# helgeanl/GP-MPC

Measured on NVIDIA H100. Metric: GP predictions/sec (N train x horizon test, fp64), higher is better.
Workload: dtype f64

## Files before the change

### gp-mpc_b200/csrc/gpmpc.cu

```cuda
#include "../../include/gpmpc.h"

#include <dlfcn.h>
#include <math.h>
#include <stdarg.h>
#include <stdlib.h>
#include <string.h>

#include <algorithm>
#include <type_traits>
#include <vector>

#include <nvtx3/nvToolsExt.h>

#include "common.cuh"
#include "gemm_dmma.cuh"
#include "predict_streamk.cuh"
#include "kernels.cuh"

#define GPMPC_VERSION 100
#define HB 64
#define NX_MAX 32
#define PSK_MAX_CTAS 2048
#define MAX_DEPTH 12
#define LOOKAHEAD_MIN_ROWS 1024
// ... 33 lines not shown
    return true;
}

template <typename T>
struct DevBuf {
    T* p = nullptr;
    size_t cap = 0;
    DevBuf() = default;
    DevBuf(const DevBuf&) = delete;
    DevBuf& operator=(const DevBuf&) = delete;
    ~DevBuf() { cudaFree(p); }
    operator T*() const { return p; }
    int ensure(gpmpc_handle_t h, long long count, const char* name);
};

struct gpmpc_handle_s {
    int N = 0, Nx = 0, Ny = 0, a0 = 0, nloc = 0, Npad = 0, device = 0;
    int nloc_max = 0;
    cudaStream_t st = nullptr;
    cudaEvent_t ev0 = nullptr, ev1 = nullptr;
    cudaStream_t sideSt[MAX_DEPTH] = {nullptr}; cudaEvent_t evA[MAX_DEPTH] = {nullptr}, evB[MAX_DEPTH] = {nullptr}, evT[MAX_DEPTH] = {nullptr}, evS[MAX_DEPTH] = {nullptr};
    long long w2off[MAX_DEPTH + 1] = {0};
    DevBuf<double> dXT, dMu, dY, dHyp, dJit, dHypTmp;
    DevBuf<double> dL, dLi, dW1, dW2;
    DevBuf<double> dAlpha, dTmp, dRes;
    DevBuf<int> dInfo;
    DevBuf<double> dKST, dPart, dPMJ, dSQ, dV, dR, dR2;
    DevBuf<unsigned int> dCnt;
    int psk_ctas = 0, opt_predict_ctas = 0;
    DevBuf<double> dCovV, dCovOut;
    DevBuf<double> dGrD;
    DevBuf<int> dGrI;
    DevBuf<double> dRm;
    DevBuf<double> dUall, dBeta, dPDV, dPH, dGradOut; bool u_valid = false;
    DevBuf<double> dDR, dVD, dPG, dPB2, dPM3, dHessOut;
    DevBuf<double> dG;
    double *dZ = nullptr, *dSigma = nullptr, *dMean = nullptr, *dVar = nullptr, *dJ = nullptr, *dCov = nullptr;
    DevBuf<double> dRoll;
    DevBuf<double> dSmV;
    DevBuf<double> dSmp;
    DevBuf<double> dIn, dOut;
    int Hcap = 0;
    double* hPinned = nullptr; double* dPinnedAlias = nullptr; size_t hPinnedBytes = 0;
    DevBuf<double> dU, dKinv, dGradPart, dGrad;
    DevBuf<double> dLoo;
    bool has_data = false, has_hyper = false, factorized = false;
    DevBuf<double> dEmTr, dEMP, dEmE, dEmF, dEmW, dEmIJ;
    DevBuf<double> dEmMeanPart, dEmPart, dEmLQ, dEmVec, dEmE2, dEmF2;
    DevBuf<double> dEmKinv, dEmGPart, dEmGRec, dEmBB; bool em_kinv_valid = false;
    std::vector<double> hyper;
    std::vector<double> logdet, yalpha;
    std::vector<int> jitter_used;
    int sms = 132;
    int opt_refine = 0, opt_small_tiles = 528;
    nccl_comm_t comm = nullptr; int rank = 0, world = 1;
    DevBuf<double> dPeerBlock; long long peerGsz = 0; int peerHcap = 0; bool peer_ready = false;
    double* peerBase[GPMPC_MAXW] = {nullptr}; bool peerOpened[GPMPC_MAXW] = {false};
    int* dPeerStatus = nullptr; int* hPeerStatus = nullptr;
    unsigned long long peer_step = 0; int opt_peer = 1; double opt_peer_timeout_s = 60.0; int clock_khz = 1980000;
    char err[512] = "";
};

static void set_error(gpmpc_handle_t h, const char* fmt, ...)
{
    va_list ap; va_start(ap, fmt);
    vsnprintf(h ? h->err : g_create_err, 512, fmt, ap);
    va_end(ap);
}

template <typename T>
int DevBuf<T>::ensure(gpmpc_handle_t h, long long count, const char* name)
{
    if ((size_t)count <= cap) return GPMPC_OK;
    if (p) {
        CUDA_TRY(cudaStreamSynchronize(h->st));
        cudaFree(p);
        p = nullptr; cap = 0;
    }
    const size_t bytes = (size_t)count * sizeof(T);
    cudaError_t e = cudaMalloc((void**)&p, bytes);
    if (e != cudaSuccess) {
        p = nullptr;
        set_error(h, "cudaMalloc(%s, %zu bytes) failed: %s", name, bytes, cudaGetErrorString(e));
        return GPMPC_ERR_CUDA;
    }
    e = cudaMemsetAsync(p, 0, bytes, h->st);
    if (e != cudaSuccess) { cudaFree(p); p = nullptr; }
    CUDA_TRY(e);
    cap = (size_t)count;
    return GPMPC_OK;
}

#define ENSURE(buf, count)                                          \
    do {                                                            \
        const int _rc = (buf).ensure(h, (long long)(count), #buf);  \
        if (_rc) return _rc;                                        \
    } while (0)

struct NvtxRange {
    explicit NvtxRange(const char* name) { nvtxRangePushA(name); }
    ~NvtxRange() { nvtxRangePop(); }
};

static inline long long slab(gpmpc_handle_t h) { return (long long)h->Npad * h->Npad; }
static inline long long w2slab(gpmpc_handle_t h) { return h->w2off[MAX_DEPTH]; }

// ... 140 lines not shown
    trmv_lower_kernel<<<g1, 256, 0, h->st>>>(Li, n, slab(h), h->dY + (long long)a * n, n,
                                              h->dTmp + (long long)a * n, n, n);
    CUDA_TRY(cudaGetLastError());
    const int nch = (n + TRT_ROWS - 1) / TRT_ROWS;
    double* P = h->dW1 + (long long)a * w2slab(h);
    dim3 g2(n / 32, nch, batch);
    trmv_lower_T_part_kernel<<<g2, 256, 0, h->st>>>(Li, n, slab(h), h->dTmp + (long long)a * n, n, P, w2slab(h), n);
    CUDA_TRY(cudaGetLastError());
    alpha_logdet_kernel<<<batch, 1024, 0, h->st>>>(P, w2slab(h), nch, h->dL + (long long)a * slab(h), n, slab(h),
                                                   h->dY + (long long)a * n, n, h->dAlpha + (long long)a * n, n, n, h->dRes + 2 * a);
    CUDA_TRY(cudaGetLastError());
    return GPMPC_OK;
}

static int factor_one(gpmpc_handle_t h, int a, const double* dHyp, double jitter, int* used)
{
    double* L = h->dL + (long long)a * slab(h);
    double* Li = h->dLi + (long long)a * slab(h);
    *used = 0;
    for (int attempt = 0; attempt < 2; ++attempt) {
        const double jit = attempt ? jitter : 0.0;
        CUDA_TRY(cudaMemcpyAsync(h->dJit + a, &jit, sizeof(double), cudaMemcpyHostToDevice, h->st));
        CUDA_TRY(cudaMemsetAsync(h->dInfo + a, 0, sizeof(int), h->st));
        {
            int rck = launch_kbuild(h, dHyp, h->dJit + a, L, 1, 0);
            if (rck) return rck;
        }
        int rc = potrf_inv_rec(h, L, Li, slab(h), slab(h), h->dInfo + a, 0, h->Npad, 1);
        if (rc) return rc;
        int info = 0;
        CUDA_TRY(cudaMemcpyAsync(&info, h->dInfo + a, sizeof(int), cudaMemcpyDeviceToHost, h->st));
        CUDA_TRY(cudaStreamSynchronize(h->st));
        if (info == 0) { *used = attempt; return GPMPC_OK; }
        *used = 1 + info;
    }
    return GPMPC_ERR_NOTPD;
}

extern "C" int gpmpc_version(void) { return GPMPC_VERSION; }

extern "C" const char* gpmpc_last_error(gpmpc_handle_t h) { return h ? h->err : g_create_err; }

extern "C" int gpmpc_destroy(gpmpc_handle_t h);

static int create_fill(gpmpc_handle_t h, int N, int N_cap, int Nx, int Ny, int out_begin, int out_count, int device)
{
    h->N = N; h->Nx = Nx; h->Ny = Ny; h->a0 = out_begin; h->nloc = out_count; h->device = device;
    h->nloc_max = out_count; h->world = 1; h->rank = 0;
    h->Npad = (std::max(N, N_cap) + GPMPC_TILE - 1) / GPMPC_TILE * GPMPC_TILE;
    CUDA_TRY(cudaSetDevice(device));
    CUDA_TRY(cudaDeviceGetAttribute(&h->sms, cudaDevAttrMultiProcessorCount, device));
    h->opt_small_tiles = 4 * h->sms;
    h->psk_ctas = PSK_CTAS_PER_SM * h->sms;
    cudaDeviceGetAttribute(&h->clock_khz, cudaDevAttrClockRate, device);
    {
        int lo = 0, hi = 0;
        cudaDeviceGetStreamPriorityRange(&lo, &hi);
        CUDA_TRY(cudaStreamCreateWithPriority(&h->st, cudaStreamNonBlocking, hi));
    }
    CUDA_TRY(cudaEventCreate(&h->ev0));
    CUDA_TRY(cudaEventCreate(&h->ev1));
    const long long np = h->Npad;
    ENSURE(h->dXT, (long long)Nx * np);
    ENSURE(h->dMu, NX_MAX);
    ENSURE(h->dY, (long long)out_count * np);
    ENSURE(h->dHyp, (long long)out_count * (Nx + 2));
    ENSURE(h->dHypTmp, Nx + 2);
    ENSURE(h->dJit, out_count);
    ENSURE(h->dL, out_count * slab(h));
    ENSURE(h->dLi, out_count * slab(h));
    {
        const int nb = h->Npad / 128;
        long long off = 0;
        for (int d = 0; d < MAX_DEPTH; ++d) {
            h->w2off[d] = off;
            const long long nd = (long long)((nb + (1 << d) - 1) >> d) * 128;
            off += nd * nd / 4 + 128;
        }
        h->w2off[MAX_DEPTH] = off;
        int lo = 0, hi = 0;
        cudaDeviceGetStreamPriorityRange(&lo, &hi);
        for (int d = 0; d < MAX_DEPTH; ++d) {
            CUDA_TRY(cudaStreamCreateWithPriority(&h->sideSt[d], cudaStreamNonBlocking, lo));
            CUDA_TRY(cudaEventCreateWithFlags(&h->evA[d], cudaEventDisableTiming));
            CUDA_TRY(cudaEventCreateWithFlags(&h->evB[d], cudaEventDisableTiming));
            CUDA_TRY(cudaEventCreateWithFlags(&h->evT[d], cudaEventDisableTiming));
            CUDA_TRY(cudaEventCreateWithFlags(&h->evS[d], cudaEventDisableTiming));
        }
    }
    ENSURE(h->dW1, out_count * w2slab(h));
    ENSURE(h->dW2, out_count * w2slab(h));
    ENSURE(h->dAlpha, (long long)out_count * np);
    ENSURE(h->dTmp, (long long)out_count * np);
    ENSURE(h->dRes, 2 * out_count);
    ENSURE(h->dInfo, out_count);
    ENSURE(h->dGrad, Nx + 2);
    h->hyper.assign((size_t)out_count * (Nx + 2), 0.0);
    h->logdet.assign(out_count, 0.0); h->yalpha.assign(out_count, 0.0); h->jitter_used.assign(out_count, 0);
    CUDA_TRY(cudaStreamSynchronize(h->st));
    return GPMPC_OK;
}


extern "C" int gpmpc_create(int N, int Nx, int Ny, int out_begin, int out_count, int device, gpmpc_handle_t* out)
{
    return gpmpc_create_reserve(N, N, Nx, Ny, out_begin, out_count, device, out);
// ... 391 lines not shown
        return GPMPC_OK;
    }
    if (!h->factorized) { set_error(h, "gpmpc_get: call gpmpc_factorize first"); return GPMPC_ERR_STATE; }
    switch (what) {
    case GPMPC_GET_CHOL: return extract_to_host(h, h->dL + (long long)al * slab(h), dst, 1);
    case GPMPC_GET_LINV: return extract_to_host(h, h->dLi + (long long)al * slab(h), dst, 1);
    case GPMPC_GET_ALPHA:
        CUDA_TRY(cudaMemcpyAsync(dst, h->dAlpha + (long long)al * h->Npad, h->N * 8, cudaMemcpyDeviceToHost, h->st));
        CUDA_TRY(cudaStreamSynchronize(h->st));
        return GPMPC_OK;
    case GPMPC_GET_LOGDET: dst[0] = h->logdet[al]; return GPMPC_OK;
    case GPMPC_GET_INVK: {
        int rc = compute_kinv(h, al);
        if (rc) return rc;
        return extract_to_host(h, h->dKinv, dst, 2);
    }
    default: set_error(h, "gpmpc_get: unknown selector %d", what); return GPMPC_ERR_ARG;
    }
}

extern "C" int gpmpc_set_option(gpmpc_handle_t h, const char* name, double value)
{
    if (!h || !name) return GPMPC_ERR_ARG;
    if (!strcmp(name, "refine")) { h->opt_refine = value != 0.0; return GPMPC_OK; }
    if (!strcmp(name, "predict_ctas")) {
        const int v = (int)value;
        if (v < 0 || v > PSK_MAX_CTAS) { set_error(h, "predict_ctas must be in [0, %d]", PSK_MAX_CTAS); return GPMPC_ERR_ARG; }
        h->opt_predict_ctas = v; return GPMPC_OK;
    }
    if (!strcmp(name, "peer_timeout_s")) { h->opt_peer_timeout_s = value > 0.0 ? value : 60.0; return GPMPC_OK; }
    if (!strcmp(name, "small_tiles")) { h->opt_small_tiles = (int)value; return GPMPC_OK; }
    if (!strcmp(name, "peer")) { h->opt_peer = value != 0.0; return GPMPC_OK; }
    set_error(h, "unknown option %s", name);
    return GPMPC_ERR_ARG;
}

static inline int ks_chunk(gpmpc_handle_t h)
{
    if (h->Npad < 8192) return 128;
    return (h->nloc >= 2 && h->Nx <= 12) ? 1024 : 512;
}

static inline int ks_blocks(gpmpc_handle_t h) { return (h->Npad + ks_chunk(h) - 1) / ks_chunk(h); }

static inline int round8(int n) { return (n + 7) / 8 * 8; }

static int ensure_rows(gpmpc_handle_t h)
{
    ENSURE(h->dV, (long long)h->nloc * HB * h->Npad);
    ENSURE(h->dR, (long long)h->nloc * HB * h->Npad);
    return GPMPC_OK;
}

static int ensure_predict_bufs(gpmpc_handle_t h, int H)
{
    const long long np = h->Npad, nt = np / 128;
    ENSURE(h->dKST, (long long)h->nloc * HB * np);
    ENSURE(h->dPMJ, (long long)h->nloc * HB * ks_blocks(h) * (h->Nx + 1));
    ENSURE(h->dSQ, (long long)h->nloc * HB * nt);
    ENSURE(h->dCnt, (long long)h->nloc * nt + h->nloc + 1);
    ENSURE(h->dPart, (long long)std::max(h->psk_ctas, h->opt_predict_ctas) * 2 * HB * PSK_BN);
    if (h->opt_refine) {
        int rc = ensure_rows(h);
        if (rc) return rc;
        ENSURE(h->dR2, (long long)h->nloc * HB * np);
    }
    if (H > h->Hcap) {
        h->Hcap = 0;
        h->dZ = h->dSigma = h->dMean = h->dVar = h->dJ = h->dCov = nullptr;
        const long long cap = std::max(H, HB);
        const int nyp = h->nloc_max * h->world;
        const long long Nx = h->Nx, Ny = h->Ny;
        ENSURE(h->dG, (long long)nyp * cap * (Nx + 2));
        ENSURE(h->dIn, cap * Nx + cap * Nx * Nx);
        ENSURE(h->dOut, cap * (2 * Ny + Ny * Nx + Ny * Ny));
        h->dZ = h->dIn; h->dSigma = h->dIn + cap * Nx;
        h->dMean = h->dOut; h->dVar = h->dOut + cap * Ny; h->dJ = h->dOut + 2 * cap * Ny;
        h->dCov = h->dOut + 2 * cap * Ny + cap * Ny * Nx;
        h->Hcap = (int)cap;
    }
    return GPMPC_OK;
}

template <int BM>
static cudaError_t psk_launch_bm(const PredictParams& p, const double* A, long long sA, const double* B, long long sB,
                                 int np, int grid, cudaStream_t st)
{
    constexpr int BYTES = psk_pipe_doubles(BM) * 8 + 2 * PSK_STAGES * 8 + 1024;
    const cudaError_t e = smem_opt_in<predict_streamk_kernel<BM>>(BYTES);
    if (e != cudaSuccess) return e;
    CUtensorMap tmA, tmB;
    if (!tmap_make(&tmA, A, np, BM, np, sA, p.nloc, BM)) return cudaErrorInvalidValue;
    if (!tmap_make(&tmB, B, np, np, np, sB, p.nloc, PSK_BN)) return cudaErrorInvalidValue;
    cudaLaunchConfig_t cfg;
    memset(&cfg, 0, sizeof(cfg));
    cfg.gridDim = dim3(grid); cfg.blockDim = dim3(PSK_THREADS); cfg.dynamicSmemBytes = BYTES; cfg.stream = st;
    cudaLaunchAttribute attr[1];
    attr[0].id = cudaLaunchAttributeProgrammaticStreamSerialization;
    attr[0].val.programmaticStreamSerializationAllowed = 1;
    cfg.attrs = attr; cfg.numAttrs = 1;
    return cudaLaunchKernelEx(&cfg, predict_streamk_kernel<BM>, p, tmA, tmB);
}

static int psk_grid(gpmpc_handle_t h, long long G)
{
    int ctas = h->opt_predict_ctas > 0 ? h->opt_predict_ctas : h->psk_ctas;
    ctas = std::min(ctas, PSK_MAX_CTAS);
    const long long by_work = std::max(1LL, G / 4);
    return (int)std::min<long long>(ctas, h->opt_predict_ctas > 0 ? G : by_work);
}

static cudaError_t psk_launch(gpmpc_handle_t h, const PredictParams& p, const double* A, const double* B)
{
    const long long sA = (long long)HB * h->Npad, sB = slab(h);
    const int np = h->Npad, grid = psk_grid(h, p.G);
    switch (round8(p.Hc)) {
    case 8: return psk_launch_bm<8>(p, A, sA, B, sB, np, grid, h->st);
    case 16: return psk_launch_bm<16>(p, A, sA, B, sB, np, grid, h->st);
    case 24: return psk_launch_bm<24>(p, A, sA, B, sB, np, grid, h->st);
    case 32: return psk_launch_bm<32>(p, A, sA, B, sB, np, grid, h->st);
    case 40: return psk_launch_bm<40>(p, A, sA, B, sB, np, grid, h->st);
    case 48: return psk_launch_bm<48>(p, A, sA, B, sB, np, grid, h->st);
    case 56: return psk_launch_bm<56>(p, A, sA, B, sB, np, grid, h->st);
    default: return psk_launch_bm<64>(p, A, sA, B, sB, np, grid, h->st);
    }
}

static void psk_base(gpmpc_handle_t h, PredictParams& p, int Hc, int upper = 0)
{
    memset(&p, 0, sizeof(p));
    const long long nt = h->Npad / 128;
    p.nloc = h->nloc; p.nt = (int)nt; p.Hc = Hc; p.upper = upper;
    p.ntb = (int)((h->Npad + PSK_BN - 1) / PSK_BN); p.nk = h->Npad / GEMM_BK;
    p.T = psk_steps_per_output(p.ntb, p.nk, upper); p.G = p.T * h->nloc;
    p.part = h->dPart;
    p.tile_cnt = h->dCnt; p.out_cnt = h->dCnt + (long long)h->nloc * nt; p.done_cnt = p.out_cnt + h->nloc;
    p.SQ = h->dSQ;
    p.hyp = h->dHyp; p.hyp_ld = h->Nx + 2; p.Nx = h->Nx;
}

static void psk_finalize(gpmpc_handle_t h, PredictParams& p, int H, int h0)
{
    p.finalize = 1; p.PMJ = h->dPMJ; p.nblk_mj = ks_blocks(h);
    p.Gloc = h->dG; p.slot0 = h->a0; p.Htot = H; p.h0 = h0;
}

static AssembleArgs assemble_args(gpmpc_handle_t h, int H, int method, const double* Sigma, int spp,
                                  double* mean, double* var, double* J, double* cov)
{
    AssembleArgs as;
    memset(&as, 0, sizeof(as));
    as.G = h->dG; as.Ny = h->Ny; as.Nx = h->Nx; as.H = H; as.method_ta = (method == GPMPC_METHOD_TA);
    as.Sigma = Sigma; as.sigma_per_point = spp;
    as.mean = mean; as.var = var; as.J = J; as.cov = cov;
    as.world = 1;
    as.stage_g = (assemble_rows_doubles(H, h->Ny, h->Nx) <= psk_pipe_doubles(round8(std::min(H, HB)))) ? 1 : 0;
    return as;
}

template <int NXP, int CH>
static cudaError_t launch_ks(gpmpc_handle_t h, const double* dZc, int Hc)
{
    const int smem = (NXP + 1) * CH * 8, nblk = ks_blocks(h);
    const cudaError_t e = smem_opt_in<ks_tile_kernel<NXP, CH>>(smem);
    if (e != cudaSuccess) return e;
    dim3 g(nblk, round8(Hc) / 8, h->nloc);
    ks_tile_kernel<NXP, CH><<<g, 256, smem, h->st>>>(h->dXT, h->Npad, h->N, h->Nx, h->dHyp, h->Nx + 2, h->dAlpha, h->Npad,
                                                     dZc, Hc, h->dKST, h->Npad, (long long)HB * h->Npad, h->dPMJ, nblk);
    return cudaGetLastError();
}

template <int CH>
static cudaError_t launch_ks_nx(gpmpc_handle_t h, const double* dZc, int Hc)
{
    const int Nx = h->Nx;
    if (Nx <= 4) return launch_ks<4, CH>(h, dZc, Hc);
    if (Nx <= 6) return launch_ks<6, CH>(h, dZc, Hc);
    if (Nx <= 8) return launch_ks<8, CH>(h, dZc, Hc);
    if (Nx <= 10) return launch_ks<10, CH>(h, dZc, Hc);
    if (Nx <= 12) return launch_ks<12, CH>(h, dZc, Hc);
    if (CH <= 512) {
        if (Nx <= 16) return launch_ks<16, (CH <= 512 ? CH : 512)>(h, dZc, Hc);
        if (Nx <= 24) return launch_ks<24, (CH <= 512 ? CH : 512)>(h, dZc, Hc);
        return launch_ks<32, (CH <= 512 ? CH : 512)>(h, dZc, Hc);
    }
    return cudaErrorInvalidValue;
}
// ... 1206 lines not shown
    CUDA_TRY(cudaIpcGetMemHandle(&mh, h->dPeerBlock));
    static_assert(sizeof(cudaIpcMemHandle_t) == 64, "IPC handle size");
    memcpy(handle64, &mh, 64);
    return GPMPC_OK;
}

extern "C" int gpmpc_peer_attach(gpmpc_handle_t h, const void* handles)
{
    if (!h || !handles) return GPMPC_ERR_ARG;
    if (!h->dPeerBlock) { set_error(h, "gpmpc_peer_attach: call gpmpc_peer_export first"); return GPMPC_ERR_STATE; }
    CUDA_TRY(cudaSetDevice(h->device));
    for (int r = 0; r < h->world; ++r) {
        if (r == h->rank) { h->peerBase[r] = h->dPeerBlock; continue; }
        cudaIpcMemHandle_t mh;
        memcpy(&mh, (const char*)handles + 64 * r, 64);
        void* ptr = nullptr;
        CUDA_TRY(cudaIpcOpenMemHandle(&ptr, mh, cudaIpcMemLazyEnablePeerAccess));
        h->peerBase[r] = (double*)ptr; h->peerOpened[r] = true;
    }
    h->peer_ready = true; h->peer_step = 0;
    return GPMPC_OK;
}

extern "C" int gpmpc_get_size(gpmpc_handle_t h, int* N, int* Nx, int* Ny)
{
    if (!h) return GPMPC_ERR_ARG;
    if (N) *N = h->N;
    if (Nx) *Nx = h->Nx;
    if (Ny) *Ny = h->Ny;
    return GPMPC_OK;
}

extern "C" void* gpmpc_stream(gpmpc_handle_t h) { return h ? (void*)h->st : nullptr; }

extern "C" int gpmpc_synchronize(gpmpc_handle_t h)
{
    if (!h) return GPMPC_ERR_ARG;
    CUDA_TRY(cudaSetDevice(h->device));
    CUDA_TRY(cudaStreamSynchronize(h->st));
    return peer_status_check(h);
}

template <typename Setup>
static int profile_product(gpmpc_handle_t h, const char* fn, int H, const double* out, bool all_outputs, int n_tail,
                           Setup&& setup, std::vector<unsigned long long>& t, int* grid)
{
    if (!h || !out || H < 1 || H > HB) return GPMPC_ERR_ARG;
    int rc = predict_guard(h, fn, GPMPC_METHOD_TA, H);
    if (rc) return rc;
    rc = predict_prepare(h, fn, HB, all_outputs);
    if (rc) return rc;
    PredictParams p;
    psk_base(h, p, H);
    *grid = psk_grid(h, p.G);
    DevBuf<unsigned long long> dbg;
    ENSURE(dbg, (long long)*grid * 2 + n_tail);
    p.dbg = dbg;
    setup(p, dbg + 2 * *grid);
    for (int rep = 0; rep < 2; ++rep) {
        const cudaError_t e = psk_launch(h, p, h->dKST, h->dLi);
        if (e != cudaSuccess) { set_error(h, "%s: %s", fn, cudaGetErrorString(e)); return GPMPC_ERR_CUDA; }
    }
    t.resize((size_t)*grid * 2 + n_tail);
    cudaMemcpyAsync(t.data(), dbg, t.size() * 8, cudaMemcpyDeviceToHost, h->st);
    cudaStreamSynchronize(h->st);
    return GPMPC_OK;
}

extern "C" int gpmpc_profile_balance(gpmpc_handle_t h, int H, double* out4)
{
    std::vector<unsigned long long> t; int grid = 0;
    const int rc = profile_product(h, __func__, H, out4, false, 0, [](PredictParams&, unsigned long long*) {}, t, &grid);
    if (rc) return rc;
    unsigned long long lo = ~0ull, hi = 0; double mn = 1e300, mx = 0.0, sum = 0.0;
    for (int c = 0; c < grid; ++c) {
        const double d = (double)(t[2 * c + 1] - t[2 * c]) * 1e-3;
        mn = std::min(mn, d); mx = std::max(mx, d); sum += d;
        lo = std::min(lo, t[2 * c]); hi = std::max(hi, t[2 * c + 1]);
    }
    out4[0] = mn; out4[1] = mx; out4[2] = sum / grid; out4[3] = (double)(hi - lo) * 1e-3;
    return GPMPC_OK;
}

extern "C" int gpmpc_profile_tail(gpmpc_handle_t h, int H, double* out8)
{
    std::vector<unsigned long long> t; int grid = 0;
    auto setup = [&](PredictParams& p, unsigned long long* tail) {
        psk_finalize(h, p, H, 0);
        p.as = assemble_args(h, H, GPMPC_METHOD_TA, h->dSigma, 0, h->dMean, h->dVar, h->dJ, h->dCov);
        p.as.dbg = tail;
        p.do_assemble = 1;
    };
    const int rc = profile_product(h, __func__, H, out8, true, 8, setup, t, &grid);
    if (rc) return rc;
    unsigned long long lo = ~0ull, hi = 0, hi2 = 0; int cmax = 0;
    for (int c = 0; c < grid; ++c) {
        lo = std::min(lo, t[2 * c]);
        if (t[2 * c + 1] > hi) { hi2 = hi; hi = t[2 * c + 1]; cmax = c; } else hi2 = std::max(hi2, t[2 * c + 1]);
    }
    for (int k = 0; k < 6; ++k) out8[k] = ((double)t[2 * grid + k] - (double)hi2) * 1e-3;
    out8[6] = (double)(hi - lo) * 1e-3;
    out8[7] = (double)(t[2 * cmax + 1] - t[2 * cmax]) * 1e-3;
    return GPMPC_OK;
}

extern "C" int gpmpc_profile_leaf(gpmpc_handle_t h, double* out15)
{
// ... 86 lines not shown
```

### gp-mpc_b200/csrc/predict_streamk.cuh

```cuda
#pragma once
#include "common.cuh"
#include "gemm_dmma.cuh"

#define GPMPC_MAXW 16
#define PSK_CW 8
#define PSK_BN (32 * PSK_CW)
#define PSK_STAGES 5
#define PSK_CTAS_PER_SM 1
#define PSK_THREADS (32 * PSK_CW)

__host__ __device__ constexpr long long psk_pipe_doubles(int bm) { return (long long)PSK_STAGES * (bm + PSK_BN) * GEMM_BK; }


struct PeerArgs {
    double* base[GPMPC_MAXW];
    int world, rank;
    long long goff;
    int flag_idx;
    unsigned long long step;
    long long timeout_clocks;
};

struct AssembleArgs {
    const double* G;
    int Ny, Nx, H, method_ta;
    const double* Sigma; int sigma_per_point;
    double *mean, *var, *J, *cov;
    const unsigned long long* flags;
    int world; unsigned long long step; int* status;
    long long timeout_clocks;
    unsigned long long* dbg;
    int stage_g;
};

struct PredictParams {
    int nloc, nt, Hc;
    int ntb, nk;
    int upper;
    long long T, G;
    double* part;
    unsigned int* tile_cnt;
    unsigned int* out_cnt;
    unsigned int* done_cnt;
    double* SQ;
    double* Vout; long long sV; int ldv;
    int finalize;
    const double* PMJ; int nblk_mj;
    const double* hyp; int hyp_ld, Nx;
    double* Gloc; int slot0, Htot, h0;
    PeerArgs pa; int use_peers, publish;
    AssembleArgs as; int do_assemble;
    unsigned long long* dbg;
};

__device__ __forceinline__ void tail_stamp(unsigned long long* dbg, int k, int tid)
{
    if (dbg && tid == 0) { unsigned long long t; asm volatile("mov.u64 %0, %%globaltimer;" : "=l"(t)); dbg[k] = t; }
}

template <bool WARP>
__device__ __forceinline__ void assemble_point(const AssembleArgs& A, int h, double* sh, int tid, int nth)
{
    const int Ny = A.Ny, Nx = A.Nx, H = A.H;
    double* Jh = sh; double* JS = sh + Ny * Nx; double* vh = sh + 2 * Ny * Nx;
    for (int idx = tid; idx < Ny * Nx; idx += nth) {
        const int a = idx / Nx, d = idx % Nx;
        const double v = __ldcg(A.G + (((long long)a) * H + h) * (Nx + 2) + 2 + d);
        Jh[idx] = v;
        if (A.J) A.J[((long long)h * Ny + a) * Nx + d] = v;
    }
    for (int a = tid; a < Ny; a += nth) {
        const double* g = A.G + (((long long)a) * H + h) * (Nx + 2);
        const double m = __ldcg(g), v = __ldcg(g + 1);
        if (A.mean) A.mean[(long long)h * Ny + a] = m;
        if (A.var) A.var[(long long)h * Ny + a] = v;
        vh[a] = v;
    }
    if (WARP) __syncwarp(); else __syncthreads();
    if (A.cov) {
        if (A.method_ta) {
            const double* Sg = A.Sigma + (A.sigma_per_point ? (long long)h * Nx * Nx : 0);
            for (int idx = tid; idx < Ny * Nx; idx += nth) {
                const int a = idx / Nx, e = idx % Nx;
                double s = 0.0;
                for (int d = 0; d < Nx; ++d) s = fma(Jh[a * Nx + d], Sg[d * Nx + e], s);
                JS[idx] = s;
            }
            if (WARP) __syncwarp(); else __syncthreads();
        }
        for (int idx = tid; idx < Ny * Ny; idx += nth) {
            const int a = idx / Ny, b = idx % Ny;
            double s = (a == b) ? vh[a] : 0.0;
// ... 136 lines not shown
}

__device__ __forceinline__ void assemble_flat(const AssembleArgs& A, double* sh, int tid, int nth)
{
    if (A.stage_g) assemble_rows(A, sh, tid, nth);
    else assemble_flat_global(A, sh, tid, nth);
}

__device__ __forceinline__ bool peer_acquire(const AssembleArgs& A, int tid, int* sh_ok)
{
    if (!A.flags) return true;
    if (tid == 0) *sh_ok = 1;
    __syncthreads();
    if (tid < A.world) {
        const long long t0 = clock64();
        unsigned long long v;
        do {
            asm volatile("ld.acquire.sys.global.u64 %0, [%1];" : "=l"(v) : "l"(A.flags + tid) : "memory");
            if (v >= A.step) break;
            if (clock64() - t0 > A.timeout_clocks) {
                *reinterpret_cast<volatile int*>(A.status) = 1 + tid;
                *reinterpret_cast<volatile int*>(sh_ok) = 0;
                break;
            }
            __nanosleep(64);
        } while (true);
    }
    __syncthreads();
    return *reinterpret_cast<volatile int*>(sh_ok) != 0;
}

__global__ void __launch_bounds__(128)
assemble_kernel(const AssembleArgs A)
{
    extern __shared__ double sh[];
    __shared__ int ok;
    if (!peer_acquire(A, threadIdx.x, &ok)) return;
    for (int h = blockIdx.x; h < A.H; h += gridDim.x) assemble_point<false>(A, h, sh, threadIdx.x, blockDim.x);
}

#define PSK_SB (PSK_BN / GEMM_BK)
__host__ __device__ inline long long psk_kstart(int ntb, int nk, int upper, int jt)
{
    const long long full = (long long)(PSK_SB / 2) * jt * (jt + 1), d = (long long)PSK_SB * ntb - nk;
    return upper ? full - jt * d : (jt == ntb ? full - d : full);
}
__host__ __device__ inline long long psk_steps_per_output(int ntb, int nk, int upper) { return psk_kstart(ntb, nk, upper, ntb); }
__device__ __forceinline__ long long psk_kstart(const PredictParams& p, int jt) { return psk_kstart(p.ntb, p.nk, p.upper, jt); }
__device__ __forceinline__ int psk_ksteps(const PredictParams& p, int jt)
{
    return p.upper ? p.nk - PSK_SB * (p.ntb - 1 - jt) : min(PSK_SB * (jt + 1), p.nk);
}

struct PskIter { int a, jt, s, ks; };

__device__ __forceinline__ void psk_iter_init(PskIter& it, long long g, const PredictParams& p)
{
    it.a = (int)(g / p.T);
    const long long r = g - (long long)it.a * p.T;
    int jt = (int)((sqrt(8.0 * (double)r / PSK_SB + 1.0) - 1.0) * 0.5);
    jt = max(0, min(jt, p.ntb - 1));
    while (jt > 0 && psk_kstart(p, jt) > r) --jt;
    while (jt + 1 < p.ntb && psk_kstart(p, jt + 1) <= r) ++jt;
    it.jt = jt; it.s = (int)(r - psk_kstart(p, jt)); it.ks = psk_ksteps(p, jt);
}
__device__ __forceinline__ void psk_iter_next(PskIter& it, const PredictParams& p)
{
    if (++it.s == it.ks) {
        it.s = 0;
        if (++it.jt == p.ntb) { it.jt = 0; ++it.a; }
        it.ks = psk_ksteps(p, it.jt);
    }
}

__device__ __forceinline__ void psk_store_record(const PredictParams& p, int a, int h, int q, double val)
{
    const long long off = (((long long)(p.slot0 + a)) * p.Htot + p.h0 + h) * (p.Nx + 2) + q;
    if (!p.use_peers) p.Gloc[off] = val;
    else for (int r = 0; r < p.pa.world; ++r) p.pa.base[r][p.pa.goff + off] = val;
}

__device__ __forceinline__ void psk_reduce_mj(const PredictParams& p, int i_begin, int i_end, int t, int nthr)
{
    const int F1 = p.Nx + 1;
    for (int i = i_begin + t; i < i_end; i += nthr) {
        const int ah = i / F1, qq = i - ah * F1, a = ah / p.Hc, h = ah - a * p.Hc;
        const double* pm = p.PMJ + ((long long)ah * p.nblk_mj) * F1 + qq;
        double s0 = 0.0, s1 = 0.0;
        int b = 0;
        for (; b + 16 <= p.nblk_mj; b += 16) {
            double v[16];
#pragma unroll
            for (int k = 0; k < 16; ++k) v[k] = __ldcg(pm + (long long)(b + k) * F1);
#pragma unroll
            for (int k = 0; k < 16; k += 2) { s0 += v[k]; s1 += v[k + 1]; }
        }
        for (; b + 2 <= p.nblk_mj; b += 2) { s0 += __ldcg(pm + (long long)b * F1); s1 += __ldcg(pm + (long long)(b + 1) * F1); }
        if (b < p.nblk_mj) s0 += __ldcg(pm + (long long)b * F1);
        psk_store_record(p, a, h, qq == 0 ? 0 : qq + 1, s0 + s1);
    }
}

__device__ __forceinline__ void psk_finalize_output(const PredictParams& p, int a, int tid, int nth)
{
    const int Nx = p.Nx;
    const double sf = p.hyp[(long long)a * p.hyp_ld + Nx];
    for (int base = 0; base < p.Hc; base += nth / 4) {
        const int h = base + (tid >> 2), j0 = tid & 3;
        double sj = 0.0;
        if (h < p.Hc) {
            const double* sq = p.SQ + ((long long)a * 64 + h) * p.nt;
            int j = j0;
            for (; j + 4 * 15 < p.nt; j += 4 * 16) {
                double v[16];
#pragma unroll
                for (int k = 0; k < 16; ++k) v[k] = __ldcg(sq + j + 4 * k);
#pragma unroll
                for (int k = 0; k < 16; ++k) sj += v[k];
            }
            for (; j < p.nt; j += 4) sj += __ldcg(sq + j);
// ... 31 lines not shown
    }
    __syncthreads();
    tail_stamp(p.as.dbg, 5, tid);
}

__global__ void __launch_bounds__(128)
sq_rows_kernel(const double* __restrict__ V, int ldv, long long sV, double* __restrict__ SQ, int nt)
{
    __shared__ double red[4];
    const int jt = blockIdx.x, h = blockIdx.y, a = blockIdx.z;
    const double v = V[(long long)a * sV + (long long)h * ldv + jt * 128 + threadIdx.x];
    const double s = warp_sum(v * v);
    if ((threadIdx.x & 31) == 0) red[threadIdx.x >> 5] = s;
    __syncthreads();
    if (threadIdx.x == 0) SQ[((long long)a * 64 + h) * nt + jt] = (red[0] + red[1]) + (red[2] + red[3]);
}

__global__ void __launch_bounds__(PSK_THREADS)
finalize_kernel(const PredictParams p)
{
    extern __shared__ double sh[];
    __shared__ unsigned int s_flag;
    __shared__ int s_ok;
    const int per = p.Hc * (p.Nx + 1);
    psk_reduce_mj(p, blockIdx.x * per, (blockIdx.x + 1) * per, threadIdx.x, PSK_THREADS);
    psk_finalize_output(p, blockIdx.x, threadIdx.x, PSK_THREADS);
    psk_step_tail(p, sh, threadIdx.x, PSK_THREADS, &s_flag, &s_ok);
}

template <int BM>
__global__ void __launch_bounds__(PSK_THREADS, PSK_CTAS_PER_SM)
predict_streamk_kernel(const PredictParams p, const __grid_constant__ CUtensorMap tmA, const __grid_constant__ CUtensorMap tmB)
{
    constexpr int BK = GEMM_BK, BN = PSK_BN, STAGES = PSK_STAGES, CW = PSK_CW, NT = PSK_THREADS;
    constexpr int NF = BM / 8;
    static_assert(BK == 16 && BN == 32 * CW && BN % 128 == 0, "one m16n8k16 per fragment and k-step, 32 L-rows per warp");
    constexpr int GR = BN / 128;
    constexpr int A_STAGE = BM * BK, B_STAGE = BN * BK;
    constexpr uint32_t STAGE_TX = (BM + BN) * BK * 8;
    static_assert(BM % 8 == 0 && BM >= 8 && BM <= 64, "BM");

    extern __shared__ __align__(16) double smem_raw[];
    double* smem = smem_align1024(smem_raw);
    double* As = smem;
    double* Bs = smem + STAGES * A_STAGE;
    uint64_t* full = reinterpret_cast<uint64_t*>(smem + STAGES * (A_STAGE + B_STAGE));
    uint64_t* empty = full + STAGES;
    __shared__ double red[BN / 16][64];
    __shared__ unsigned int s_flag;
    __shared__ int s_ok;

    const int tid = threadIdx.x, warp = tid >> 5, lane = tid & 31, g = lane >> 2, t = lane & 3;
    const long long C = gridDim.x, c = blockIdx.x;
    const long long g0 = p.G * c / C;
    const int nsteps = (int)(p.G * (c + 1) / C - g0);
    if (nsteps <= 0) return;
    if (p.dbg && threadIdx.x == 0) { unsigned long long t0; asm volatile("mov.u64 %0, %%globaltimer;" : "=l"(t0)); p.dbg[2 * blockIdx.x] = t0; }

    __shared__ PskIter s_pit;
    __shared__ int s_pg;
    __shared__ uint64_t s_pol[2];
    if (tid == 0) {
#pragma unroll
        for (int s = 0; s < STAGES; ++s) { mbar_init(full + s, 1); mbar_init(empty + s, CW); }
        mbar_fence_init();
    }
    __syncthreads();

    auto issue = [&]() {
        PskIter it = s_pit;
        const int pg = s_pg, s = pg % STAGES;
        if (pg >= STAGES) mbar_wait(empty + s, (uint32_t)(((pg / STAGES) - 1) & 1));
        mbar_arrive_expect_tx(full + s, STAGE_TX);
        const int jta = p.upper ? p.ntb - 1 - it.jt : it.jt;
        const int k0 = (p.upper ? jta * BN : 0) + it.s * BK;
        tma_tile_g2s_3d_hint(As + s * A_STAGE, &tmA, k0, 0, it.a, full + s, s_pol[1]);
        tma_tile_g2s_3d_hint(Bs + s * B_STAGE, &tmB, k0, jta * BN, it.a, full + s, s_pol[0]);
        psk_iter_next(it, p);
        s_pit = it;
        s_pg = pg + 1;
    };
    constexpr int AHEAD = STAGES - 2;
    asm volatile("griddepcontrol.wait;" ::: "memory");
    if (tid == 0) {
        PskIter it;
        psk_iter_init(it, g0, p);
        s_pit = it; s_pg = 0;
        s_pol[0] = l2_policy_evict_first(); s_pol[1] = l2_policy_evict_last();
#pragma unroll
        for (int s = 0; s < AHEAD; ++s)
            if (s_pg < nsteps) issue();
    }
    if (p.finalize) {
        const int tot = p.nloc * p.Hc * (p.Nx + 1), per = (tot + (int)C - 1) / (int)C;
        if (tid >= 32) {
            psk_reduce_mj(p, min(tot, (int)c * per), min(tot, ((int)c + 1) * per), tid - 32, NT - 32);
            if (p.use_peers) __threadfence_system();
        }
    }

    PskIter cit;
    psk_iter_init(cit, g0, p);
    int cj[4];
#pragma unroll
    for (int j = 0; j < 4; ++j) cj[j] = (((j + 4 * (t >> 1)) ^ g) << 1) + (t & 1);
    int i = 0;
    while (i < nsteps) {
        const int a = cit.a, jt = cit.jt, s_begin = cit.s, ksteps = cit.ks;
        const int seg = min(ksteps - s_begin, nsteps - i);
        const int hh = warp / (128 / 32);
        const int st_lo = p.upper ? (128 / BK) * hh : 0;
        const int st_hi = p.upper ? ksteps : PSK_SB * jt + (128 / BK) * (hh + 1);
        double acc[2][NF][4];
#pragma unroll
        for (int mi = 0; mi < 2; ++mi)
#pragma unroll
            for (int ni = 0; ni < NF; ++ni)
#pragma unroll
                for (int r = 0; r < 4; ++r) acc[mi][ni][r] = 0.0;

        for (int q = 0; q < seg; ++q, ++i) {
            const int s = i % STAGES;
            if (tid == 0 && i + AHEAD < nsteps) issue();
            mbar_wait(full + s, (uint32_t)((i / STAGES) & 1));
            const int st = s_begin + q;
            if (st >= st_lo && st < st_hi) {
                const double* ls = Bs + s * B_STAGE + (warp * 32 + g) * 16;
                const double* ps = As + s * A_STAGE + g * 16;
                double av[2][8];
#pragma unroll
                for (int mi = 0; mi < 2; ++mi)
#pragma unroll
                    for (int j = 0; j < 4; ++j) { av[mi][2 * j] = ls[256 * mi + cj[j]]; av[mi][2 * j + 1] = ls[256 * mi + 128 + cj[j]]; }
#pragma unroll
                for (int ni = 0; ni < NF; ++ni) {
                    double bv[4];
#pragma unroll
                    for (int j = 0; j < 4; ++j) bv[j] = ps[ni * 8 * 16 + cj[j]];
                    dmma16816(acc[0][ni], av[0], bv);
                    dmma16816(acc[1][ni], av[1], bv);
                }
            }
            __syncwarp();
            if (lane == 0) mbar_arrive(empty + s);
        }
        cit.s = s_begin + seg - 1;
        psk_iter_next(cit, p);

        bool have_tile = true;
        if (seg != ksteps) {
            const long long tg0 = (long long)a * p.T + psk_kstart(p, jt), tg1 = tg0 + ksteps;
            const long long Cf = gridDim.x;
            const int c_first = (int)(((tg0 + 1) * Cf - 1) / p.G), c_last = (int)((tg1 * Cf - 1) / p.G);
            double2* mine = reinterpret_cast<double2*>(p.part + ((long long)blockIdx.x * 2 + (s_begin == 0 ? 1 : 0)) * (BM * BN)) + tid;
#pragma unroll
            for (int mi = 0; mi < 2; ++mi)
#pragma unroll
                for (int ni = 0; ni < NF; ++ni)
#pragma unroll
                    for (int hf = 0; hf < 2; ++hf)
                        __stcg(mine + ((mi * NF + ni) * 2 + hf) * NT, make_double2(acc[mi][ni][2 * hf], acc[mi][ni][2 * hf + 1]));
            __threadfence();
            __syncthreads();
            if (tid == 0) {
                unsigned int* cnt = p.tile_cnt + (long long)a * p.ntb + jt;
                const unsigned int old = atomicAdd(cnt, 1u);
                const unsigned int last = (old == (unsigned int)(c_last - c_first)) ? 1u : 0u;
                if (last) *cnt = 0u;
                s_flag = last;
            }
            __syncthreads();
            have_tile = s_flag != 0u;
            if (have_tile) {
                __threadfence();
#pragma unroll
                for (int mi = 0; mi < 2; ++mi)
#pragma unroll
                    for (int ni = 0; ni < NF; ++ni)
#pragma unroll
                        for (int r = 0; r < 4; ++r) acc[mi][ni][r] = 0.0;
                for (int cc = c_first; cc <= c_last; ++cc) {
                    const double2* src = reinterpret_cast<const double2*>(p.part + ((long long)cc * 2 + (cc == c_first ? 1 : 0)) * (BM * BN)) + tid;
#pragma unroll
                    for (int mi = 0; mi < 2; ++mi)
#pragma unroll
                        for (int ni = 0; ni < NF; ++ni)
#pragma unroll
                            for (int hf = 0; hf < 2; ++hf) {
                                const double2 v = __ldcg(src + ((mi * NF + ni) * 2 + hf) * NT);
                                acc[mi][ni][2 * hf] += v.x; acc[mi][ni][2 * hf + 1] += v.y;
                            }
                }
            }
        }
        if (!have_tile) continue;

        const int jta = p.upper ? p.ntb - 1 - jt : jt;
        const int row0 = jta * BN + warp * 32;
        if (p.Vout && row0 < p.nk * BK) {
            double* vo = p.Vout + (long long)a * p.sV + row0 + g;
#pragma unroll
            for (int mi = 0; mi < 2; ++mi)
#pragma unroll
                for (int ni = 0; ni < NF; ++ni)
#pragma unroll
                    for (int r = 0; r < 4; ++r)
                        vo[(long long)(ni * 8 + 2 * t + (r & 1)) * p.ldv + 16 * mi + 8 * (r >> 1)] = acc[mi][ni][r];
        }
#pragma unroll
        for (int mi = 0; mi < 2; ++mi)
#pragma unroll
            for (int ni = 0; ni < NF; ++ni)
#pragma unroll
                for (int j = 0; j < 2; ++j) {
                    double r = acc[mi][ni][j] * acc[mi][ni][j];
                    r = fma(acc[mi][ni][j + 2], acc[mi][ni][j + 2], r);
                    r += __shfl_xor_sync(0xffffffffu, r, 4);
                    r += __shfl_xor_sync(0xffffffffu, r, 8);
                    r += __shfl_xor_sync(0xffffffffu, r, 16);
                    if (g == 0) red[2 * warp + mi][ni * 8 + 2 * t + j] = r;
                }
        __syncthreads();
        for (int idx = tid; idx < GR * BM; idx += NT) {
            const int gr = idx / BM, pt = idx - gr * BM, col = jta * GR + gr;
            if (col < p.nt) {
                double r = 0.0;
#pragma unroll
                for (int b = 0; b < 8; ++b) r += red[8 * gr + b][pt];
                __stcg(p.SQ + ((long long)a * 64 + pt) * p.nt + col, r);
            }
        }
        __threadfence();
        __syncthreads();
        if (tid == 0) {
            unsigned int* cnt = p.out_cnt + a;
// ... 17 lines not shown
```

Baseline: 14770.

## Split stream-K predict work into L2-sized rounds of outputs

Partitions the stream-K prediction GEMM into rounds, each covering only as many outputs as fit in about two-thirds of L2, and distributes each round's steps across all CTAs. The aim is to keep the per-output A/B panels resident in L2 while the CTAs sweep them, instead of streaming all outputs at once. Partial-sum buffers grow by the number of rounds, and each round adds extra stream-K fixup boundaries, which raises reduction and iteration overhead. When all outputs fit in a single round, behaviour matches the previous schedule.

```diff
diff --git a/gp-mpc_b200/csrc/gpmpc.cu b/gp-mpc_b200/csrc/gpmpc.cu
--- a/gp-mpc_b200/csrc/gpmpc.cu
+++ b/gp-mpc_b200/csrc/gpmpc.cu
@@ -109,6 +109,7 @@
     std::vector<double> logdet, yalpha;
     std::vector<int> jitter_used;
     int sms = 132;
+    long long l2_bytes = 50LL << 20;
     int opt_refine = 0, opt_small_tiles = 528;
     nccl_comm_t comm = nullptr; int rank = 0, world = 1;
     DevBuf<double> dPeerBlock; long long peerGsz = 0; int peerHcap = 0; bool peer_ready = false;
@@ -355,6 +356,11 @@
     CUDA_TRY(cudaDeviceGetAttribute(&h->sms, cudaDevAttrMultiProcessorCount, device));
     h->opt_small_tiles = 4 * h->sms;
     h->psk_ctas = PSK_CTAS_PER_SM * h->sms;
+    {
+        int l2 = 0;
+        CUDA_TRY(cudaDeviceGetAttribute(&l2, cudaDevAttrL2CacheSize, device));
+        h->l2_bytes = l2;
+    }
     cudaDeviceGetAttribute(&h->clock_khz, cudaDevAttrClockRate, device);
     {
         int lo = 0, hi = 0;
@@ -852,6 +858,13 @@
     return GPMPC_OK;
 }
 
+static int psk_round_outputs(gpmpc_handle_t h)
+{
+    const long long per_output = (long long)HB * h->Npad * 8;
+    return (int)std::max(1LL, std::min<long long>(h->nloc, 2 * h->l2_bytes / 3 / per_output));
+}
+static int psk_rounds(gpmpc_handle_t h) { const int R = psk_round_outputs(h); return (h->nloc + R - 1) / R; }
+
 static int ensure_predict_bufs(gpmpc_handle_t h, int H)
 {
     const long long np = h->Npad, nt = np / 128;
@@ -859,7 +872,7 @@
     ENSURE(h->dPMJ, (long long)h->nloc * HB * ks_blocks(h) * (h->Nx + 1));
     ENSURE(h->dSQ, (long long)h->nloc * HB * nt);
     ENSURE(h->dCnt, (long long)h->nloc * nt + h->nloc + 1);
-    ENSURE(h->dPart, (long long)std::max(h->psk_ctas, h->opt_predict_ctas) * 2 * HB * PSK_BN);
+    ENSURE(h->dPart, (long long)std::max(h->psk_ctas, h->opt_predict_ctas) * psk_rounds(h) * 2 * HB * PSK_BN);
     if (h->opt_refine) {
         int rc = ensure_rows(h);
         if (rc) return rc;
@@ -902,8 +915,9 @@
     return cudaLaunchKernelEx(&cfg, predict_streamk_kernel<BM>, p, tmA, tmB);
 }
 
-static int psk_grid(gpmpc_handle_t h, long long G)
-{
+static int psk_grid(gpmpc_handle_t h, const PredictParams& p)
+{
+    const long long G = p.T * p.R;
     int ctas = h->opt_predict_ctas > 0 ? h->opt_predict_ctas : h->psk_ctas;
     ctas = std::min(ctas, PSK_MAX_CTAS);
     const long long by_work = std::max(1LL, G / 4);
@@ -913,7 +927,7 @@
 static cudaError_t psk_launch(gpmpc_handle_t h, const PredictParams& p, const double* A, const double* B)
 {
     const long long sA = (long long)HB * h->Npad, sB = slab(h);
-    const int np = h->Npad, grid = psk_grid(h, p.G);
+    const int np = h->Npad, grid = psk_grid(h, p);
     switch (round8(p.Hc)) {
     case 8: return psk_launch_bm<8>(p, A, sA, B, sB, np, grid, h->st);
     case 16: return psk_launch_bm<16>(p, A, sA, B, sB, np, grid, h->st);
@@ -932,7 +946,8 @@
     const long long nt = h->Npad / 128;
     p.nloc = h->nloc; p.nt = (int)nt; p.Hc = Hc; p.upper = upper;
     p.ntb = (int)((h->Npad + PSK_BN - 1) / PSK_BN); p.nk = h->Npad / GEMM_BK;
-    p.T = psk_steps_per_output(p.ntb, p.nk, upper); p.G = p.T * h->nloc;
+    p.T = psk_steps_per_output(p.ntb, p.nk, upper);
+    p.R = psk_round_outputs(h); p.rounds = psk_rounds(h);
     p.part = h->dPart;
     p.tile_cnt = h->dCnt; p.out_cnt = h->dCnt + (long long)h->nloc * nt; p.done_cnt = p.out_cnt + h->nloc;
     p.SQ = h->dSQ;
@@ -2245,7 +2260,7 @@
     if (rc) return rc;
     PredictParams p;
     psk_base(h, p, H);
-    *grid = psk_grid(h, p.G);
+    *grid = psk_grid(h, p);
     DevBuf<unsigned long long> dbg;
     ENSURE(dbg, (long long)*grid * 2 + n_tail);
     p.dbg = dbg;
diff --git a/gp-mpc_b200/csrc/predict_streamk.cuh b/gp-mpc_b200/csrc/predict_streamk.cuh
--- a/gp-mpc_b200/csrc/predict_streamk.cuh
+++ b/gp-mpc_b200/csrc/predict_streamk.cuh
@@ -37,7 +37,8 @@
     int nloc, nt, Hc;
     int ntb, nk;
     int upper;
-    long long T, G;
+    long long T;
+    int R, rounds;
     double* part;
     unsigned int* tile_cnt;
     unsigned int* out_cnt;
@@ -280,9 +281,12 @@
     return p.upper ? p.nk - PSK_SB * (p.ntb - 1 - jt) : min(PSK_SB * (jt + 1), p.nk);
 }
 
-struct PskIter { int a, jt, s, ks; };
-
-__device__ __forceinline__ void psk_iter_init(PskIter& it, long long g, const PredictParams& p)
+__device__ __forceinline__ long long psk_round_steps(const PredictParams& p, int r) { return (long long)min(p.R, p.nloc - r * p.R) * p.T; }
+__device__ __forceinline__ long long psk_round_ctas(long long steps) { return min((long long)gridDim.x, steps); }
+
+struct PskIter { int a, jt, s, ks, r, n; };
+
+__device__ __forceinline__ void psk_iter_at(PskIter& it, long long g, const PredictParams& p)
 {
     it.a = (int)(g / p.T);
     const long long r = g - (long long)it.a * p.T;
@@ -292,8 +296,32 @@
     while (jt + 1 < p.ntb && psk_kstart(p, jt + 1) <= r) ++jt;
     it.jt = jt; it.s = (int)(r - psk_kstart(p, jt)); it.ks = psk_ksteps(p, jt);
 }
+__device__ __forceinline__ void psk_iter_round(PskIter& it, const PredictParams& p, int r)
+{
+    const long long c = blockIdx.x;
+    for (; r < p.rounds; ++r) {
+        const long long Gr = psk_round_steps(p, r), Cr = psk_round_ctas(Gr);
+        if (c >= Cr) continue;
+        const long long g0 = Gr * c / Cr;
+        psk_iter_at(it, (long long)r * p.R * p.T + g0, p);
+        it.r = r; it.n = (int)(Gr * (c + 1) / Cr - g0);
+        return;
+    }
+    it.r = p.rounds; it.n = 0;
+}
+__device__ __forceinline__ long long psk_cta_steps(const PredictParams& p)
+{
+    const long long c = blockIdx.x;
+    long long n = 0;
+    for (int r = 0; r < p.rounds; ++r) {
+        const long long Gr = psk_round_steps(p, r), Cr = psk_round_ctas(Gr);
+        if (c < Cr) n += Gr * (c + 1) / Cr - Gr * c / Cr;
+    }
+    return n;
+}
 __device__ __forceinline__ void psk_iter_next(PskIter& it, const PredictParams& p)
 {
+    if (--it.n == 0) { psk_iter_round(it, p, it.r + 1); return; }
     if (++it.s == it.ks) {
         it.s = 0;
         if (++it.jt == p.ntb) { it.jt = 0; ++it.a; }
@@ -431,8 +459,7 @@
 
     const int tid = threadIdx.x, warp = tid >> 5, lane = tid & 31, g = lane >> 2, t = lane & 3;
     const long long C = gridDim.x, c = blockIdx.x;
-    const long long g0 = p.G * c / C;
-    const int nsteps = (int)(p.G * (c + 1) / C - g0);
+    const int nsteps = (int)psk_cta_steps(p);
     if (nsteps <= 0) return;
     if (p.dbg && threadIdx.x == 0) { unsigned long long t0; asm volatile("mov.u64 %0, %%globaltimer;" : "=l"(t0)); p.dbg[2 * blockIdx.x] = t0; }
 
@@ -463,7 +490,7 @@
     asm volatile("griddepcontrol.wait;" ::: "memory");
     if (tid == 0) {
         PskIter it;
-        psk_iter_init(it, g0, p);
+        psk_iter_round(it, p, 0);
         s_pit = it; s_pg = 0;
         s_pol[0] = l2_policy_evict_first(); s_pol[1] = l2_policy_evict_last();
 #pragma unroll
@@ -479,14 +506,14 @@
     }
 
     PskIter cit;
-    psk_iter_init(cit, g0, p);
+    psk_iter_round(cit, p, 0);
     int cj[4];
 #pragma unroll
     for (int j = 0; j < 4; ++j) cj[j] = (((j + 4 * (t >> 1)) ^ g) << 1) + (t & 1);
     int i = 0;
     while (i < nsteps) {
-        const int a = cit.a, jt = cit.jt, s_begin = cit.s, ksteps = cit.ks;
-        const int seg = min(ksteps - s_begin, nsteps - i);
+        const int a = cit.a, jt = cit.jt, s_begin = cit.s, ksteps = cit.ks, r = cit.r;
+        const int seg = min(ksteps - s_begin, cit.n);
         const int hh = warp / (128 / 32);
         const int st_lo = p.upper ? (128 / BK) * hh : 0;
         const int st_hi = p.upper ? ksteps : PSK_SB * jt + (128 / BK) * (hh + 1);
@@ -523,15 +550,16 @@
             __syncwarp();
             if (lane == 0) mbar_arrive(empty + s);
         }
-        cit.s = s_begin + seg - 1;
+        cit.s = s_begin + seg - 1; cit.n -= seg - 1;
         psk_iter_next(cit, p);
 
         bool have_tile = true;
         if (seg != ksteps) {
-            const long long tg0 = (long long)a * p.T + psk_kstart(p, jt), tg1 = tg0 + ksteps;
-            const long long Cf = gridDim.x;
-            const int c_first = (int)(((tg0 + 1) * Cf - 1) / p.G), c_last = (int)((tg1 * Cf - 1) / p.G);
-            double2* mine = reinterpret_cast<double2*>(p.part + ((long long)blockIdx.x * 2 + (s_begin == 0 ? 1 : 0)) * (BM * BN)) + tid;
+            const long long Gr = psk_round_steps(p, r), Cr = psk_round_ctas(Gr);
+            const long long tg0 = (long long)(a - r * p.R) * p.T + psk_kstart(p, jt), tg1 = tg0 + ksteps;
+            const int c_first = (int)(((tg0 + 1) * Cr - 1) / Gr), c_last = (int)((tg1 * Cr - 1) / Gr);
+            const long long slot0 = (long long)r * 2;
+            double2* mine = reinterpret_cast<double2*>(p.part + ((long long)blockIdx.x * p.rounds * 2 + slot0 + (s_begin == 0 ? 1 : 0)) * (BM * BN)) + tid;
 #pragma unroll
             for (int mi = 0; mi < 2; ++mi)
 #pragma unroll
@@ -559,7 +587,7 @@
 #pragma unroll
                         for (int r = 0; r < 4; ++r) acc[mi][ni][r] = 0.0;
                 for (int cc = c_first; cc <= c_last; ++cc) {
-                    const double2* src = reinterpret_cast<const double2*>(p.part + ((long long)cc * 2 + (cc == c_first ? 1 : 0)) * (BM * BN)) + tid;
+                    const double2* src = reinterpret_cast<const double2*>(p.part + ((long long)cc * p.rounds * 2 + slot0 + (cc == c_first ? 1 : 0)) * (BM * BN)) + tid;
 #pragma unroll
                     for (int mi = 0; mi < 2; ++mi)
 #pragma unroll
```

Result: faster. 14990, median of 6 (+1.5%).
